# MarineRoboticsGroup/mac

Measured on AMD Instinct MI355X. Metric: frank_wolfe_iters_per_sec, higher is better.
Workload: dtype f64; 1 GPU; configs[3]: ER N=100000 ~2M candidates, chain fixed, K=10%; N=100000, m_candidates=2001737, K=200173, fixed_edges=99999, fw_iters=209, parallelism=single GPU

## Files before the change

include/machip.h:

```cpp
#ifndef MACHIP_H
#define MACHIP_H

#include <stdint.h>

#ifdef __cplusplus
extern "C" {
#endif

#define MACHIP_ABI_VERSION 16

typedef enum machip_status {
    MACHIP_OK = 0,
    MACHIP_NOT_CONVERGED = 1,
    MACHIP_DISCONNECTED = 2,
    MACHIP_BAD_ARG = 3,
    MACHIP_HIP_ERROR = 4,
    MACHIP_RCCL_ERROR = 5,
    MACHIP_NO_DEVICE = 6
} machip_status;

typedef struct machip_problem machip_problem;

typedef struct machip_solve_stats {
    int64_t lanczos_steps;
    int64_t spmv_total;
    int64_t vec_passes;
    int64_t restarts;
    int64_t nnz;
    int64_t support;
    double residual;
    double lnorm;
    double gpu_ms;
// ... 66 lines not shown
int machip_comm_mode(machip_problem* p);
int machip_shard_plan(int64_t m, int nranks, int rank, int64_t* lo, int64_t* hi, int64_t* shard);

int machip_eval_batch(machip_problem* p, int B, const double* X, double tol, int max_steps, double* lambda2,
                      int* status);

int machip_fw_sweep(machip_problem* p, int B, const int64_t* ks, const double* X0, int max_iters, double gap_tol,
                    double grad_tol, double tol, int max_steps, int warm_start, int round_decimals, double* X_out,
                    double* R_out, double* upper, double* f_traj, int* iters, int* status);

int machip_set_solver(machip_problem* p, int mode);

int machip_set_precision(machip_problem* p, int precision);

#define MACHIP_OPTION_AUTO INT64_MIN
int machip_set_option(machip_problem* p, const char* name, int64_t value);
int machip_get_option(machip_problem* p, const char* name, int64_t* value);
const char* machip_option_name(int i);

int machip_synchronize(machip_problem* p);

int machip_membench(int device, int64_t bytes, int reps, double* read_gbs, double* triad_gbs);
int machip_panel_plan(int64_t n, int64_t nnz, int maxlen, int* out12);
void machip_release_cache(void);
int machip_host_tridiag_smallest(const double* a, const double* b, int J, double* theta, double* s);
int machip_host_follow_records(const double* tri3, int J, int n, double e_target, double tiny_l, int jcap, int* points, int cap,
                               int* npoints, int* jeff, double* est);

typedef struct machip_esp machip_esp;
#define MACHIP_ESP_DENSE_INVERSE 1
#define MACHIP_ESP_MATRIX_FREE 2
#define MACHIP_ESP_SPANNING_TREE 8
#define MACHIP_ESP_EDGE_RELAX 16
#define MACHIP_ESP_EDGE_RELAX_TREE 32
int machip_esp_create(int device, int64_t n, int64_t n_fixed, const int32_t* fi, const int32_t* fj, const double* fw,
                      int64_t m, const int32_t* ci, const int32_t* cj, const double* cw, int fold, int flags, machip_esp** out);
void machip_esp_destroy(machip_esp* h);
int machip_esp_select(machip_esp* h, int nb, const int64_t* ks, int32_t* order_out, double* gain_out, double* t_ms_out);
int machip_esp_weighted_resistances(machip_esp* h, double* r_out);
int machip_esp_info(machip_esp* h, int32_t* info4, double* beta);
int machip_esp_tree_plan(int64_t n, int64_t n_fixed, const int32_t* fi, const int32_t* fj, const double* fw, int32_t* parent,
                         double* R, int32_t* pre, int32_t* end, int64_t* n_seeds, int32_t* su, int32_t* sv, double* sw);
int machip_esp_seeds(machip_esp* h, int64_t* seeds_out);

int machip_esp_relax_eval(machip_esp* h, const double* x, double* F_out, double* grad_out);
int machip_esp_relax_run(machip_esp* h, int64_t k, int max_iters, double gap_tol, double grad_tol, double* x_inout,
// ... 28 lines not shown
```

mac_amd/_lib.py:

```python
from __future__ import annotations

import ctypes as C
import os

import numpy as np

_HERE = os.path.dirname(os.path.abspath(__file__))
LIB_PATH = os.environ.get("MACHIP_LIB") or os.path.join(_HERE, "libmachip.so")

OK, NOT_CONVERGED, DISCONNECTED, BAD_ARG, HIP_ERROR, RCCL_ERROR, NO_DEVICE = range(7)
STATUS_NAMES = ["OK", "NOT_CONVERGED", "DISCONNECTED", "BAD_ARG", "HIP_ERROR", "RCCL_ERROR", "NO_DEVICE"]


class MachipError(RuntimeError):
    def __init__(self, status, msg):
        super().__init__(f"libmachip: {STATUS_NAMES[status] if 0 <= status < 7 else status}: {msg}")
        self.status = status


class NotConverged(MachipError):
    pass


class Disconnected(MachipError):
# ... 52 lines not shown
    "machip_comm_init_ipc": (C.c_int, [C.c_void_p, C.c_int, C.c_int, C.c_void_p, C.c_double]),
    "machip_comm_close_ipc": (C.c_int, [C.c_void_p]),
    "machip_comm_mode": (C.c_int, [C.c_void_p]),
    "machip_shard_plan": (C.c_int, [C.c_int64, C.c_int, C.c_int, C.POINTER(C.c_int64), C.POINTER(C.c_int64), C.POINTER(C.c_int64)]),
    "machip_eval_batch": (C.c_int, [C.c_void_p, C.c_int, _f64p, C.c_double, C.c_int, _f64p, C.POINTER(C.c_int)]),
    "machip_fw_sweep": (C.c_int, [C.c_void_p, C.c_int, C.POINTER(C.c_int64), _f64p, C.c_int, C.c_double, C.c_double, C.c_double,
                                  C.c_int, C.c_int, C.c_int, _f64p, _f64p, _f64p, _f64p, C.POINTER(C.c_int), C.POINTER(C.c_int)]),
    "machip_set_solver": (C.c_int, [C.c_void_p, C.c_int]),
    "machip_set_option": (C.c_int, [C.c_void_p, C.c_char_p, C.c_int64]),
    "machip_get_option": (C.c_int, [C.c_void_p, C.c_char_p, C.POINTER(C.c_int64)]),
    "machip_option_name": (C.c_char_p, [C.c_int]),
    "machip_comm_drop_ipc": (C.c_int, [C.c_void_p]),
    "machip_comm_drop": (C.c_int, [C.c_void_p]),
    "machip_comm_timing": (C.c_int, [C.c_void_p, _f64p, _f64p]),
    "machip_solve_mode": (C.c_int, [C.c_void_p, C.POINTER(C.c_int64)]),
    "machip_set_precision": (C.c_int, [C.c_void_p, C.c_int]),
    "machip_synchronize": (C.c_int, [C.c_void_p]),
    "machip_membench": (C.c_int, [C.c_int, C.c_int64, C.c_int, _f64p, _f64p]),
    "machip_host_tridiag_smallest": (C.c_int, [_f64p, _f64p, C.c_int, _f64p, _f64p]),
    "machip_host_follow_records": (C.c_int, [_f64p, C.c_int, C.c_int, C.c_double, C.c_double, C.c_int, C.POINTER(C.c_int), C.c_int,
                                             C.POINTER(C.c_int), C.POINTER(C.c_int), C.POINTER(C.c_double)]),
    "machip_release_cache": (None, []),
    "machip_panel_plan": (C.c_int, [C.c_int64, C.c_int64, C.c_int, C.POINTER(C.c_int)]),
    "machip_esp_create": (C.c_int, [C.c_int, C.c_int64, C.c_int64, _i32p, _i32p, _f64p, C.c_int64, _i32p, _i32p, _f64p,
                                    C.c_int, C.c_int, C.POINTER(C.c_void_p)]),
    "machip_esp_destroy": (None, [C.c_void_p]),
    "machip_esp_select": (C.c_int, [C.c_void_p, C.c_int, C.POINTER(C.c_int64), _i32p, _f64p, _f64p]),
    "machip_esp_weighted_resistances": (C.c_int, [C.c_void_p, _f64p]),
    "machip_esp_info": (C.c_int, [C.c_void_p, _i32p, C.POINTER(C.c_double)]),
    "machip_esp_tree_plan": (C.c_int, [C.c_int64, C.c_int64, _i32p, _i32p, _f64p, _i32p, _f64p, _i32p, _i32p, C.POINTER(C.c_int64),
                                       _i32p, _i32p, _f64p]),
    "machip_esp_seeds": (C.c_int, [C.c_void_p, C.POINTER(C.c_int64)]),
    "machip_esp_relax_eval": (C.c_int, [C.c_void_p, _f64p, C.POINTER(C.c_double), _f64p]),
    "machip_esp_relax_run": (C.c_int, [C.c_void_p, C.c_int64, C.c_int, C.c_double, C.c_double, _f64p, _f64p, _f64p, _f64p,
                                       C.POINTER(C.c_int), C.POINTER(C.c_double)]),
    "machip_esp_relax_inner": (C.c_int, [C.c_void_p, _f64p, _f64p, C.POINTER(C.c_double)]),
    "machip_esp_relax_info": (C.c_int, [C.c_void_p, _i32p]),
    "machip_esp_relax_gram": (C.c_int, [C.c_void_p, _f64p, C.c_int64]),
    "machip_esp_exchange": (C.c_int, [C.c_void_p, C.c_int64, _i32p, C.c_int64, C.c_double, _i32p, _i32p, _i32p, _f64p,
                                      C.POINTER(C.c_int64), C.POINTER(C.c_int32), _f64p]),
    "machip_esp_exchange_edge": (C.c_int, [C.c_void_p, C.c_int64, _i32p, C.c_int64, C.c_double, _i32p, _i32p, _i32p, _f64p,
                                           C.POINTER(C.c_int64), C.POINTER(C.c_int32), _f64p]),
    "machip_eig_create": (C.c_int, [C.c_int, C.c_int64, C.c_int64, _i32p, _i32p, _f64p, C.c_int64, _i32p, _i32p, _f64p,
                                    C.c_int, C.c_int, C.c_int, C.POINTER(C.c_void_p)]),
    "machip_eig_destroy": (None, [C.c_void_p]),
    "machip_eig_select": (C.c_int, [C.c_void_p, C.c_int64, _i32p, _f64p, _f64p]),
# ... 550 lines not shown
        os.dup2(2, 1)

    def __exit__(self, *exc):
        os.dup2(self._saved, 1)
        os.close(self._saved)


def _single_node_bootstrap():
    os.environ.setdefault("NCCL_SOCKET_IFNAME", "lo")


def comm_init_local(problems):
    lib = load()
    arr = (C.c_void_p * len(problems))(*[p._h for p in problems])
    check(lib.machip_comm_init_local(arr, len(problems)))


def shard_plan(m, nranks, rank):
    lo, hi, sh = C.c_int64(), C.c_int64(), C.c_int64()
    check(load().machip_shard_plan(int(m), int(nranks), int(rank), C.byref(lo), C.byref(hi), C.byref(sh)))
    return int(lo.value), int(hi.value), int(sh.value)


def comm_unique_id() -> bytes:
    _single_node_bootstrap()
    buf = C.create_string_buffer(128)
    lib = load()
    with _stdout_to_stderr():
        st = lib.machip_comm_unique_id(buf)
    check(st)
    return buf.raw


def fiedler_csr(indptr, indices, data, n, tol=1e-8, max_steps=0, x0=None, q=0, device=0):
    lib = load()
    indptr, indices, data = i32(indptr), i32(indices), f64(data)
    lam = C.c_double()
    v = np.empty(n)
    X = np.empty((q, n)) if q else None
    x0a = f64(x0) if x0 is not None else None
    stats = SolveStats()
    check(lib.machip_fiedler_csr(int(device), int(n), p_i32(indptr), p_i32(indices), p_f64(data), float(tol),
                                 int(max_steps), p_f64(x0a), C.byref(lam), p_f64(v), p_f64(X), int(q),
                                 C.byref(stats)))
    return lam.value, v, (X.T if X is not None else None), stats

# ... 23 lines not shown
```

mac_amd/csrc/kernels.h:

```cpp
#pragma once
#include "common.h"

namespace machip {

template <typename T>
struct CsrViewT {
    int n;
    const int* rowptr;
    const int* col;
    const T* val;
};
using CsrView = CsrViewT<double>;

struct PatternView {
    int n;
    const int* prow;
    const int* pcol;
    const int* pk;
    const double* pw;
};

struct LanState {
    int jA;
    int jB;
// ... 5 lines not shown
    int n;
    LanState* st;
    double* u;
    double* w;
    double* V;
    double* alpha;
    double* beta;
    double* l1;
    double* part_u;
    int P_u;
    double* part_a;
    int P_a;
};

constexpr int kAsmGrid = 4096;
__global__ __launch_bounds__(kBlock) void k_x_bits(const double* __restrict__ x, long m, double tol, unsigned long long* __restrict__ bits) {
    for (long i = (long)blockIdx.x * kBlock + threadIdx.x; i < m; i += (long)gridDim.x * kBlock) {
        const unsigned long long bal = __ballot(x[i] > tol);
        if ((threadIdx.x & 63) == 0) bits[i >> 6] = bal;
    }
}
__device__ __forceinline__ bool x_bit(const unsigned int* __restrict__ bits32, int k) { return (bits32[k >> 5] >> (k & 31)) & 1u; }

template <int G>
__global__ __launch_bounds__(kBlock) void k_asm_count(PatternView P, const unsigned int* __restrict__ xbits,
                                                      int rows_per_block,
                                                      int* __restrict__ cnt, int* __restrict__ blk_sum,
                                                      int* __restrict__ hsum = nullptr) {
    __shared__ int sm[4];
    constexpr int GPB = kBlock / G;
    const int lane = threadIdx.x % G, g = threadIdx.x / G;
    const int r0 = blockIdx.x * rows_per_block;
    const int r1 = min(P.n, r0 + rows_per_block);
    int local = 0, supp = 0, mx = 0;
    for (int r = r0 + g; r < r1; r += GPB) {
        const int b = P.prow[r], e = P.prow[r + 1];
        int c = 0, sc = 0;
        for (int p = b + lane; p < e; p += G) {
            const int k = P.pk[p];
            const bool cand = k >= 0;
            const bool act = cand ? x_bit(xbits, k) : true;
            c += act;
            sc += (cand && act);
        }
        c = group_sum_i<G>(c);
        sc = group_sum_i<G>(sc);
        if (lane == 0) {
            cnt[r] = c + 1;
            local += c + 1;
            supp += sc;
            mx = max(mx, c + 1);
        }
    }
    const int tot = block_sum_i(local, sm);
    const int stot = block_sum_i(supp, sm);
#pragma unroll
    for (int o = 32; o > 0; o >>= 1) mx = max(mx, __shfl_xor(mx, o, kWave));
    __syncthreads();
    if ((threadIdx.x & 63) == 0) sm[threadIdx.x >> 6] = mx;
    __syncthreads();
    if (threadIdx.x == 0) {
        blk_sum[blockIdx.x] = tot;
        blk_sum[kAsmGrid + blockIdx.x] = stot;
        const int longest = max(max(sm[0], sm[1]), max(sm[2], sm[3]));
        blk_sum[2 * kAsmGrid + blockIdx.x] = longest;
        if (hsum) {
            hsum[blockIdx.x] = tot; hsum[kAsmGrid + blockIdx.x] = stot; hsum[2 * kAsmGrid + blockIdx.x] = longest;
        }
    }
}

struct PanSpec {
    int NP = 0;
    int C = 1;
    int band = 0;
    int* ps = nullptr;
    double* bd = nullptr;
    int* bpk = nullptr;
    int* ovf = nullptr;
};

template <int G>
__global__ __launch_bounds__(kBlock) void k_asm_fill(PatternView P, const unsigned int* __restrict__ xbits, const double* __restrict__ x,
                                                     int rows_per_block,
                                                     const int* __restrict__ cnt,
                                                     const int* __restrict__ blk_sum,
                                                     int* __restrict__ rowptr, int* __restrict__ col,
                                                     double* __restrict__ val,
                                                     double* __restrict__ blk_lnorm, PanSpec S = PanSpec()) {
    extern __shared__ __attribute__((aligned(16))) char smem_raw[];
    int* s_off = reinterpret_cast<int*>(smem_raw);
    __shared__ int sm_i[4];
    __shared__ double sm_d[4];
    __shared__ int s_chunk[kBlock];
    constexpr int GPB = kBlock / G;
    const int tid = threadIdx.x;
    const int lane = tid % G, g = tid / G;
    const int r0 = blockIdx.x * rows_per_block;
    const int r1 = min(P.n, r0 + rows_per_block);
    const int nr = max(0, r1 - r0);

    int acc = 0;
    for (int b = tid; b < (int)blockIdx.x; b += kBlock) acc += blk_sum[b];
    const int base = block_sum_i(acc, sm_i);

    const int per = (nr + kBlock - 1) / kBlock;
    int csum = 0;
    for (int i = 0; i < per; ++i) {
        const int idx = tid * per + i;
        if (idx < nr) csum += cnt[r0 + idx];
    }
    {
        const int ln = tid & 63, wv = tid >> 6;
        int x = csum;
        for (int o = 1; o < 64; o <<= 1) { const int y = __shfl_up(x, o, kWave); if (ln >= o) x += y; }
        if (ln == 63) s_chunk[wv] = x;
        __syncthreads();
        int before = 0;
        for (int q = 0; q < wv; ++q) before += s_chunk[q];
        int run = before + x - csum;
        if (tid == kBlock - 1) s_off[nr] = before + x;
        for (int i = 0; i < per; ++i) {
            const int idx = tid * per + i;
            if (idx < nr) { s_off[idx] = run; run += cnt[r0 + idx]; }
        }
    }
    __syncthreads();

    double lmax = 0.0;
    for (int r = r0 + g; r < r1; r += GPB) {
        const int b = P.prow[r], e = P.prow[r + 1];
        const int out = base + s_off[r - r0];
        int pos = out + 1;
        double dsum = 0.0, asum = 0.0;
        int lastpid = 0;
        int hb = 0x7fffffff, hn = 0;
        double vl = 0.0, vu = 0.0;
        const int gbase = ((tid & 63) / G) * G;
        for (int p0 = b; p0 < e; p0 += G) {
            const int p = p0 + lane;
            const bool in = p < e;
            const int kc = in ? P.pk[p] : -1;
            const double wgt = in ? P.pw[p] : 0.0;
            const double xk = kc >= 0 ? x[kc] : 1.0;
            const bool act = in && (kc < 0 || x_bit(xbits, kc));
            const double v = act ? xk * wgt : 0.0;
            const unsigned long long bal = __ballot(act);
            unsigned long long gm;
            if (G == 64) gm = bal;
            else gm = (bal >> gbase) & ((1ull << (G & 63)) - 1ull);
            const unsigned long long below = gm & ((1ull << lane) - 1ull);
            const int before = __popcll(below);
            const int c = act ? P.pcol[p] : 0;
            if (act) { col[pos + before] = c; val[pos + before] = -v; }
            if (S.NP) {
                const int pid = act ? c / S.C : 0;
                const int src = below ? 63 - __builtin_clzll(below) : 0;
                const int got = __shfl(pid, gbase + src, kWave);
                const int ppid = below ? got : lastpid;
                if (act) {
                    const int q = pos + before;
                    for (int pp = ppid + 1; pp <= pid; ++pp) S.ps[(size_t)r * (S.NP + 1) + pp] = q;
                    if (S.band && (c == r - 1 || c == r + 1)) {
                        hb = min(hb, q); hn += 1;
                        if (c == r - 1) vl += -v; else vu += -v;
                    }
                }
                if (gm) lastpid = __shfl(pid, gbase + 63 - __builtin_clzll(gm), kWave);
            }
            pos += __popcll(gm);
            dsum += v;
            asum += fabs(v);
        }
        dsum = group_sum<G>(dsum);
        asum = group_sum<G>(asum);
        if (S.NP) {
            if (lane == 0) S.ps[(size_t)r * (S.NP + 1)] = out + 1;
            for (int pp = lastpid + 1 + lane; pp <= S.NP; pp += G) S.ps[(size_t)r * (S.NP + 1) + pp] = pos;
            if (S.band) {
                hn = group_sum_i<G>(hn);
                vl = group_sum<G>(vl); vu = group_sum<G>(vu);
#pragma unroll
                for (int o = G / 2; o > 0; o >>= 1) hb = min(hb, __shfl_xor(hb, o, kWave));
                if (lane == 0) {
                    S.bpk[r] = ((hn ? hb : pos) << 3) | min(hn, 7);
                    if (hn > 7) *S.ovf = 1;
                    S.bd[r] = dsum; S.bd[(size_t)P.n + r] = vl; S.bd[2 * (size_t)P.n + r] = vu;
                }
            }
        }
        if (lane == 0) {
            rowptr[r] = out;
            col[out] = r;
            val[out] = dsum;
            lmax = fmax(lmax, fabs(dsum) + asum);
        }
    }
    lmax = block_max(lmax, sm_d);
    if (tid == 0) {
        blk_lnorm[blockIdx.x] = lmax;
        if (blockIdx.x == gridDim.x - 1) rowptr[P.n] = base + s_off[nr];
    }
}

template <int G, class Op>
__device__ __forceinline__ void spmv_rows_vec(const CsrView& A, const double* __restrict__ x, Op& op) {
    constexpr int GPB = kBlock / G;
    const int lane = threadIdx.x % G, g = threadIdx.x / G;
    const int stride = gridDim.x * GPB;
    for (int r = blockIdx.x * GPB + g; r < A.n; r += 2 * stride) {
        const int r2 = r + stride;
        const bool two = r2 < A.n;
        const int b = A.rowptr[r], e = A.rowptr[r + 1];
        const int b2 = two ? A.rowptr[r2] : 0, e2 = two ? A.rowptr[r2 + 1] : 0;
        double acc = 0.0, acc2 = 0.0;
        int p = b + lane, q = b2 + lane;
        while (p < e || q < e2) {
            double v1 = 0.0, x1 = 0.0, v2 = 0.0, x2 = 0.0;
            if (p < e) { v1 = A.val[p]; x1 = op.gather(x, A.col[p]); }
            if (q < e2) { v2 = A.val[q]; x2 = op.gather(x, A.col[q]); }
            if (p < e) acc += v1 * x1;
            if (q < e2) acc2 += v2 * x2;
            p += G; q += G;
        }
// ... 1155 lines not shown
```

mac_amd/csrc/machip.hip:

```cpp
#include <rccl/rccl.h>
#include <unistd.h>

#include <algorithm>
#include <atomic>
#include <cmath>
#include <chrono>
#include <condition_variable>
#include <functional>
#include <future>
#include <memory>
#include <mutex>
#include <numeric>
#include <thread>
#include <vector>

#include "solver.h"
#include "esp.h"
#include "esp_free.h"
#include "esp_tree.h"
#include "esp_select.h"
#include "esp_relax.h"
#include "esp_exchange.h"
#include "esp_exchange_edge.h"
#include "eig.h"
// ... 47 lines not shown
        if (broken) return false;
        const unsigned long gen = generation;
        if (++waiting == nranks) { waiting = 0; ++generation; cv.notify_all(); return true; }
        cv.wait(lk, [&] { return generation != gen || broken; });
        return !broken;
    }
    void abort() {
        std::lock_guard<std::mutex> lk(mu);
        broken = true;
        cv.notify_all();
    }
};

struct machip_problem {
    int device = 0;
    hipStream_t stream = nullptr;
    int n = 0;
    long m = 0, m_pad = 0;
    double tol_sel = 1e-10;
    int *prow = nullptr, *pcol = nullptr, *pk = nullptr;
    double* pw = nullptr;
    long P = 0;
    int asm_G = 16, asm_rpb = 1, asm_grid = 1;
    int *ci = nullptr, *cj = nullptr;
    double* cw = nullptr;
    double *x = nullptr, *x_next = nullptr, *g = nullptr, *s = nullptr, *scratch_m = nullptr;
    int *cnt = nullptr, *blk_sum = nullptr, *rowptr = nullptr, *col = nullptr;
    double *val = nullptr, *blk_lnorm = nullptr;
    unsigned long long *xb = nullptr, *xb_next = nullptr;
    bool xb_valid = false, xb_next_valid = false;
    long nnz = 0, support = 0;
    int maxlen = 0;
    double lnorm = 0.0;
    bool assembled = false, have_vec = false, csr_only = false;
    bool band_dups_ok = true;
    unsigned int* hist = nullptr;
    SelState* sel = nullptr;
    double* part_fw = nullptr;
    int* h_int = nullptr;
    double* h_dbl = nullptr;
    int* d_hint = nullptr;
    double* d_hdbl = nullptr;
    Solver sol;
    ncclComm_t comm = nullptr;
    std::shared_ptr<LocalGroup> lgroup;
    bool first_collective_pending = false;
    hipEvent_t ev_g0 = nullptr, ev_g1 = nullptr, ev_g2 = nullptr;
    bool ev_g_valid = false;
    std::unique_ptr<IpcGroup> ipcg;
    int rank = 0, nranks = 1;
// ... 12 lines not shown
        if (hipGetDeviceProperties(&prop, device) == hipSuccess && prop.multiProcessorCount > 0) {
            const int words = (prop.multiProcessorCount + 31) / 32;
            std::vector<uint32_t> mask((size_t)words, 0xffffffffu);
            if (prop.multiProcessorCount % 32) mask.back() = (1u << (prop.multiProcessorCount % 32)) - 1u;
            if (hipExtStreamCreateWithCUMask(out, (uint32_t)words, mask.data()) == hipSuccess) return MACHIP_OK;
            (void)hipGetLastError();
        }
    }
    HIP_TRY(hipStreamCreateWithFlags(out, hipStreamNonBlocking));
    return MACHIP_OK;
}

namespace {

std::mutex g_csr_mu;
machip_problem* g_csr_cache = nullptr;

struct Slot {
    int col;
    int k;
    double w;
};

int build_pattern(machip_problem* p, int64_t nf, const int32_t* fi, const int32_t* fj, const double* fw,
                  int64_t m, const int32_t* ci, const int32_t* cj, const double* cw) {
    const Options& opt = p->sol.opt;
    const int n = p->n;
    std::vector<long> deg((size_t)n + 1, 0);
    auto chk = [&](int a, int b) { return a >= 0 && a < n && b >= 0 && b < n; };
    for (int64_t e = 0; e < nf; ++e) {
        if (!chk(fi[e], fj[e])) return fail(MACHIP_BAD_ARG, "fixed edge endpoint out of range");
        if (fi[e] != fj[e]) { deg[(size_t)fi[e]]++; deg[(size_t)fj[e]]++; }
    }
    for (int64_t e = 0; e < m; ++e) {
        if (!chk(ci[e], cj[e])) return fail(MACHIP_BAD_ARG, "candidate edge endpoint out of range");
        if (ci[e] != cj[e]) { deg[(size_t)ci[e]]++; deg[(size_t)cj[e]]++; }
    }
    std::vector<long> off((size_t)n + 1, 0);
    for (int r = 0; r < n; ++r) off[(size_t)r + 1] = off[(size_t)r] + deg[(size_t)r];
    std::vector<Slot> slots((size_t)off[(size_t)n]);
    std::vector<long> cur(off.begin(), off.end() - 1);
    for (int64_t e = 0; e < nf; ++e) {
        const int a = fi[e], b = fj[e];
        if (a == b) continue;
        slots[(size_t)cur[(size_t)a]++] = Slot{b, -1, fw[e]};
        slots[(size_t)cur[(size_t)b]++] = Slot{a, -1, fw[e]};
// ... 33 lines not shown
    }
    p->P = (long)pcol.size();
    ST_TRY(dev_alloc(&p->prow, (size_t)n + 1));
    ST_TRY(dev_alloc(&p->pcol, (size_t)p->P)); ST_TRY(dev_alloc(&p->pk, (size_t)p->P)); ST_TRY(dev_alloc(&p->pw, (size_t)p->P));
    HIP_TRY(hipMemcpyAsync(p->prow, prow.data(), sizeof(int) * ((size_t)n + 1), hipMemcpyHostToDevice, p->stream));
    if (p->P) {
        HIP_TRY(hipMemcpyAsync(p->pcol, pcol.data(), sizeof(int) * (size_t)p->P, hipMemcpyHostToDevice, p->stream));
        HIP_TRY(hipMemcpyAsync(p->pk, pk.data(), sizeof(int) * (size_t)p->P, hipMemcpyHostToDevice, p->stream));
        HIP_TRY(hipMemcpyAsync(p->pw, pw.data(), sizeof(double) * (size_t)p->P, hipMemcpyHostToDevice, p->stream));
    }
    HIP_TRY(hipStreamSynchronize(p->stream));
    const double mean = n ? (double)p->P / n : 1.0;
    int G = 4;
    while (G < 64 && G < mean * 0.75) G <<= 1;
    p->asm_G = OPT(asm_g, G);
    const int gpb = kBlock / p->asm_G;
    long nblk = std::min<long>(std::min(kAsmGrid, std::max(1, OPT(asm_maxgrid, kAsmGrid))), ((long)n + gpb - 1) / gpb);
    if (nblk < 1) nblk = 1;
    long rpb = ((long)n + nblk - 1) / nblk;
    rpb = (rpb + gpb - 1) / gpb * gpb;
    p->asm_rpb = (int)rpb;
    p->asm_grid = (int)(((long)n + rpb - 1) / rpb);
    if (p->asm_grid < 1) p->asm_grid = 1;
    if ((rpb + 1) * (long)sizeof(int) > 64 * 1024)
        return fail(MACHIP_BAD_ARG, "num_nodes above the supported 16.7 million (row-offset scan of the assembly kernel)");
    return MACHIP_OK;
}

template <int G>
void launch_asm(machip_problem* p, const PanSpec& S) {
    const PatternView P = p->pattern();
    const unsigned int* xb32 = reinterpret_cast<const unsigned int*>(p->xb);
    k_asm_count<G><<<p->asm_grid, kBlock, 0, p->stream>>>(P, xb32, p->asm_rpb, p->cnt, p->blk_sum, p->d_hint);
    const size_t lds = sizeof(int) * ((size_t)p->asm_rpb + 1);
    k_asm_fill<G><<<p->asm_grid, kBlock, lds, p->stream>>>(P, xb32, p->x, p->asm_rpb, p->cnt, p->blk_sum,
                                                           p->rowptr, p->col, p->val, p->d_hdbl, S);
}

int assemble(machip_problem* p) {
    if (p->csr_only) return fail(MACHIP_BAD_ARG, "handle wraps a caller CSR; nothing to assemble");
    PanSpec S;
    ST_TRY(p->sol.pan_spec_prepare(&S));
    if (!p->xb_valid) {
        const int grid = std::max(1, (int)std::min<long>(kMaxGrid, (p->m + kBlock - 1) / kBlock));
        k_x_bits<<<grid, kBlock, 0, p->stream>>>(p->x, p->m, p->tol_sel, p->xb);
        p->xb_valid = true;
    }
    switch (p->asm_G) {
        case 4: launch_asm<4>(p, S); break;
        case 8: launch_asm<8>(p, S); break;
        case 16: launch_asm<16>(p, S); break;
        case 32: launch_asm<32>(p, S); break;
        default: launch_asm<64>(p, S); break;
    }
    HIP_TRY(hipGetLastError());
    const int gb = p->asm_grid;
    HIP_TRY(hipStreamSynchronize(p->stream));
    long nnz = 0, supp = 0;
    int maxlen = 0;
    double ln = 0.0;
    for (int b = 0; b < gb; ++b) {
        nnz += p->h_int[b]; supp += p->h_int[kAsmGrid + b]; maxlen = std::max(maxlen, p->h_int[2 * kAsmGrid + b]);
        ln = std::max(ln, p->h_dbl[b]);
    }
    p->nnz = nnz; p->support = supp / 2; p->lnorm = ln; p->maxlen = maxlen;
    p->assembled = true;
    return MACHIP_OK;
}

int alloc_common(machip_problem* p, int vbudget_mb = 0) {
    ST_TRY(p->sol.init(p->n, p->stream, vbudget_mb));
    HIP_TRY(hipHostMalloc((void**)&p->h_int, sizeof(int) * 3 * kAsmGrid, hipHostMallocMapped));
    HIP_TRY(hipHostMalloc((void**)&p->h_dbl, sizeof(double) * std::max(4 * kMaxGrid, kAsmGrid), hipHostMallocMapped));
    HIP_TRY(hipHostGetDevicePointer((void**)&p->d_hint, p->h_int, 0));
    HIP_TRY(hipHostGetDevicePointer((void**)&p->d_hdbl, p->h_dbl, 0));
    return MACHIP_OK;
}

int select_on(machip_problem* p, const double* keys, long k, SelState* st, int prefer_high, bool hist0_done = false) {
    const Options& opt = p->sol.opt;
    const long m = p->m;
    if (k < 0) k = 0;
    if (k > m) k = m;
    if (m <= kSelSmallMax && OPT(sel_small, 1)) {
        k_sel_small<<<1, 1024, 0, p->stream>>>(keys, m, (long long)k, st, prefer_high);
        HIP_TRY(hipGetLastError());
        return MACHIP_OK;
// ... 188 lines not shown
    HIP_TRY(hipSetDevice(device));
    machip_problem* p = new machip_problem();
    p->device = device;
    p->n = (int)n;
    p->m = (long)m;
    p->m_pad = (long)m;
    p->tol_sel = min_sel_tol;
    int st = MACHIP_OK;
    auto body = [&]() -> int {
        HIP_TRY(hipStreamCreateWithFlags(&p->stream, hipStreamNonBlocking));
        ST_TRY(build_pattern(p, n_fixed, fi, fj, fw, m, ci, cj, cw));
        const size_t mp = (size_t)m + 64 * 8;
        ST_TRY(dev_alloc(&p->ci, mp)); ST_TRY(dev_alloc(&p->cj, mp)); ST_TRY(dev_alloc(&p->cw, mp));
        ST_TRY(dev_alloc(&p->x, mp)); ST_TRY(dev_alloc(&p->x_next, mp)); ST_TRY(dev_alloc(&p->g, mp)); ST_TRY(dev_alloc(&p->s, mp));
        if (m) {
            HIP_TRY(hipMemcpyAsync(p->ci, ci, sizeof(int) * (size_t)m, hipMemcpyHostToDevice, p->stream));
            HIP_TRY(hipMemcpyAsync(p->cj, cj, sizeof(int) * (size_t)m, hipMemcpyHostToDevice, p->stream));
            HIP_TRY(hipMemcpyAsync(p->cw, cw, sizeof(double) * (size_t)m, hipMemcpyHostToDevice, p->stream));
        }
        HIP_TRY(hipMemsetAsync(p->x, 0, sizeof(double) * mp, p->stream));
        HIP_TRY(hipMemsetAsync(p->g, 0, sizeof(double) * mp, p->stream));
        HIP_TRY(hipStreamSynchronize(p->stream));
        const size_t cap = (size_t)p->P + (size_t)n + 8;
        ST_TRY(dev_alloc(&p->cnt, (size_t)n + 1)); ST_TRY(dev_alloc(&p->blk_sum, 3 * kAsmGrid));
        ST_TRY(dev_alloc(&p->rowptr, (size_t)n + 1)); ST_TRY(dev_alloc(&p->col, cap)); ST_TRY(dev_alloc(&p->val, cap));
        ST_TRY(dev_alloc(&p->blk_lnorm, kAsmGrid));
        ST_TRY(dev_alloc(&p->xb, (size_t)m / 64 + 2)); ST_TRY(dev_alloc(&p->xb_next, (size_t)m / 64 + 2));
        ST_TRY(dev_alloc(&p->hist, (6 + kSelRep) * kBins)); ST_TRY(dev_alloc(&p->sel, 2)); ST_TRY(dev_alloc(&p->part_fw, 2 * kMaxGrid));
        ST_TRY(alloc_common(p));
        p->sol.csr_cap = cap;
        p->sol.pat = p->pattern();
        p->sol.pan_allowed = p->band_dups_ok;
        {
            std::vector<char> has((size_t)n, 0);
            for (int64_t e = 0; e < n_fixed; ++e) {
                const int a = std::min(fi[e], fj[e]), b = std::max(fi[e], fj[e]);
                if (a >= 0 && b < n && b == a + 1 && fw[e] > 0.0) has[(size_t)a] = 1;
            }
            long cnt = 0;
            for (int64_t i = 0; i + 1 < n; ++i) cnt += has[(size_t)i];
            p->sol.chain_like = cnt >= (long)(0.98 * (double)(n - 1));
            p->sol.chain_edges = cnt;
        }
        return MACHIP_OK;
    };
    st = body();
    if (st != MACHIP_OK) { machip_destroy(p); return st; }
    *out = p;
    return MACHIP_OK;
}

void machip_destroy(machip_problem* p) {
    if (!p) return;
    for (machip_problem* q : p->lanes) machip_destroy(q);
    p->lanes.clear();
    (void)hipSetDevice(p->device);
    if (p->stream) (void)hipStreamSynchronize(p->stream);
    if (p->is_lane) { p->prow = p->pcol = p->pk = nullptr; p->pw = nullptr; p->ci = p->cj = nullptr; p->cw = nullptr; }
    if (p->comm) (void)ncclCommDestroy(p->comm);
    if (p->lgroup) p->lgroup->abort();
    if (p->ipcg) {
        IpcGroup& G = *p->ipcg;
        if (!G.clean_exit) { k_ipc_abort<<<1, 64, 0, p->stream>>>(G.view); (void)hipStreamSynchronize(p->stream); }
        p->sol.ipc = nullptr;
        p->ipcg.reset();
    }
    p->sol.destroy();
    void* ptrs[] = {p->prow, p->pcol, p->pk, p->pw, p->ci, p->cj, p->cw, p->x, p->x_next, p->g, p->s, p->scratch_m, p->cnt,
                    p->blk_sum, p->rowptr, p->col, p->val, p->blk_lnorm, p->xb, p->xb_next, p->hist, p->sel, p->part_fw};
    for (void* q : ptrs) if (q) (void)hipFree(q);
    for (hipEvent_t e : {p->ev_g0, p->ev_g1, p->ev_g2}) if (e) (void)hipEventDestroy(e);
    if (p->h_int) (void)hipHostFree(p->h_int);
    if (p->h_dbl) (void)hipHostFree(p->h_dbl);
    if (p->stream) (void)hipStreamDestroy(p->stream);
    delete p;
}

int machip_set_x(machip_problem* p, const double* x) {
    if (!p || !x || p->csr_only) return fail(MACHIP_BAD_ARG, "machip_set_x: bad handle or NULL x");
    HIP_TRY(hipSetDevice(p->device));
    HIP_TRY(hipMemcpyAsync(p->x, x, sizeof(double) * (size_t)p->m, hipMemcpyHostToDevice, p->stream));
    HIP_TRY(hipStreamSynchronize(p->stream));
    p->assembled = false; p->xb_valid = false;
    return MACHIP_OK;
}

int machip_get_x(machip_problem* p, double* x) {
    if (!p || !x || p->csr_only) return fail(MACHIP_BAD_ARG, "machip_get_x: bad handle or NULL x");
    HIP_TRY(hipSetDevice(p->device));
    HIP_TRY(hipMemcpyAsync(x, p->x, sizeof(double) * (size_t)p->m, hipMemcpyDeviceToHost, p->stream));
    HIP_TRY(hipStreamSynchronize(p->stream));
    return MACHIP_OK;
// ... 513 lines not shown
    return 0;
}

int machip_panel_plan(int64_t n, int64_t nnz, int maxlen, int* out12) {
    if (n < 1 || n > 2000000000ll || nnz < 0 || !out12) return fail(MACHIP_BAD_ARG, "machip_panel_plan: bad argument");
    const Options& opt = default_options();
    const PanPlan pp = plan_panel(opt, (int)n, (long)nnz, maxlen, true, -1, false, OPT(stream, 1) != 0);
    out12[0] = pp.on ? 1 : 0; out12[1] = pp.NP; out12[2] = pp.C; out12[3] = pp.NB; out12[4] = pp.NTB; out12[5] = pp.TWW; out12[6] = pp.RPT; out12[7] = pp.grid2;
    out12[8] = pp.u ? 1 : 0; out12[9] = pp.LPT; out12[10] = pp.TWT; out12[11] = pp.cells;
    return MACHIP_OK;
}

#ifdef PAN_CLOCKS
extern "C" int machip_debug_pan_clocks(machip_problem* p, long long* out, int groups) {
    if (!p || !out || groups < 1 || groups > kMaxGrid || !p->sol.panv.clk) return fail(MACHIP_BAD_ARG, "machip_debug_pan_clocks: no clock buffer");
    HIP_TRY(hipSetDevice(p->device));
    HIP_TRY(hipStreamSynchronize(p->stream));
    HIP_TRY(hipMemcpy(out, p->sol.panv.clk, sizeof(long long) * 16 * (size_t)groups, hipMemcpyDeviceToHost));
    HIP_TRY(hipMemset(p->sol.panv.clk, 0, sizeof(long long) * 16 * (size_t)kMaxGrid));
    return MACHIP_OK;
}
#endif

int machip_shard_plan(int64_t m, int nranks, int rank, int64_t* lo, int64_t* hi, int64_t* shard) {
    if (m < 0 || nranks < 1 || rank < 0 || rank >= nranks || !lo || !hi || !shard) return fail(MACHIP_BAD_ARG, "machip_shard_plan: bad argument");
    long a, b, c;
    shard_plan((long)m, nranks, rank, &a, &b, &c);
    *lo = a; *hi = b; *shard = c;
    return MACHIP_OK;
}

namespace {
int make_lane(machip_problem* p, machip_problem** out) {
    machip_problem* q = new machip_problem();
    q->is_lane = true;
    q->device = p->device; q->n = p->n; q->m = p->m; q->m_pad = p->m; q->tol_sel = p->tol_sel;
    q->prow = p->prow; q->pcol = p->pcol; q->pk = p->pk; q->pw = p->pw; q->P = p->P;
    q->asm_G = p->asm_G; q->asm_rpb = p->asm_rpb; q->asm_grid = p->asm_grid;
    q->ci = p->ci; q->cj = p->cj; q->cw = p->cw;
    auto body = [&]() -> int {
        ST_TRY(create_lane_stream(p->sol.opt, q->device, &q->stream));
        ST_TRY(dev_alloc(&q->x, (size_t)q->m + 64));
        const size_t cap = (size_t)q->P + (size_t)q->n + 8;
        ST_TRY(dev_alloc(&q->cnt, (size_t)q->n + 1)); ST_TRY(dev_alloc(&q->blk_sum, 3 * kAsmGrid));
        ST_TRY(dev_alloc(&q->rowptr, (size_t)q->n + 1)); ST_TRY(dev_alloc(&q->col, cap)); ST_TRY(dev_alloc(&q->val, cap));
        ST_TRY(dev_alloc(&q->blk_lnorm, kAsmGrid));
        ST_TRY(dev_alloc(&q->xb, (size_t)q->m / 64 + 2)); ST_TRY(dev_alloc(&q->xb_next, (size_t)q->m / 64 + 2));
        const Options& opt = p->sol.opt;
        q->sol.opt = opt;
        ST_TRY(alloc_common(q, std::max(16, OPT(lane_vbudget_mb, std::max(16, OPT(vbudget_mb, 4096) / 8)))));
        q->sol.csr_cap = cap;
        q->sol.pat = q->pattern();
        q->sol.pan_allowed = p->sol.pan_allowed;
        q->sol.chain_like = p->sol.chain_like; q->sol.chain_edges = p->sol.chain_edges;
        return MACHIP_OK;
    };
    const int st = body();
    if (st != MACHIP_OK) { machip_destroy(q); return st; }
    *out = q;
    return MACHIP_OK;
}

int ensure_lane_fw(machip_problem* q) {
    if (q->lane_fw_ready) return MACHIP_OK;
    const size_t mp = (size_t)q->m + 64 * 8;
    if (!q->x_next) ST_TRY(dev_alloc(&q->x_next, mp));
    if (!q->g) ST_TRY(dev_alloc(&q->g, mp));
// ... 569 lines not shown
```

Before: 133.7 iter/s.

## Replace per-row count pass with slot bitmask and prefix marks in assembly

The count kernel now scans pattern slots linearly, producing a per-64-slot active bitmask and word prefix counts instead of per-row counts. The fill kernel derives each row's output offset and each entry's position from these marks with popcount, removing the large row-offset shared-memory scan and its node-count limit. Fill also unrolls two slot groups per iteration, prefetches the next row's bounds, and computes longest-row stats itself. This trades row-granular counting for slot-granular bitmasks, adding extra mark lookups per entry during fill.

```diff
diff --git a/include/machip.h b/include/machip.h
--- a/include/machip.h
+++ b/include/machip.h
@@ -7,7 +7,7 @@
 extern "C" {
 #endif
 
-#define MACHIP_ABI_VERSION 16
+#define MACHIP_ABI_VERSION 17
 
 typedef enum machip_status {
     MACHIP_OK = 0,
@@ -120,6 +120,7 @@
 
 int machip_membench(int device, int64_t bytes, int reps, double* read_gbs, double* triad_gbs);
 int machip_panel_plan(int64_t n, int64_t nnz, int maxlen, int* out12);
+int machip_asm_mark_plan(int64_t slots, int* out3);
 void machip_release_cache(void);
 int machip_host_tridiag_smallest(const double* a, const double* b, int J, double* theta, double* s);
 int machip_host_follow_records(const double* tri3, int J, int n, double e_target, double tiny_l, int jcap, int* points, int cap,
diff --git a/mac_amd/_lib.py b/mac_amd/_lib.py
--- a/mac_amd/_lib.py
+++ b/mac_amd/_lib.py
@@ -98,6 +98,7 @@
                                              C.POINTER(C.c_int), C.POINTER(C.c_int), C.POINTER(C.c_double)]),
     "machip_release_cache": (None, []),
     "machip_panel_plan": (C.c_int, [C.c_int64, C.c_int64, C.c_int, C.POINTER(C.c_int)]),
+    "machip_asm_mark_plan": (C.c_int, [C.c_int64, C.POINTER(C.c_int)]),
     "machip_esp_create": (C.c_int, [C.c_int, C.c_int64, C.c_int64, _i32p, _i32p, _f64p, C.c_int64, _i32p, _i32p, _f64p,
                                     C.c_int, C.c_int, C.POINTER(C.c_void_p)]),
     "machip_esp_destroy": (None, [C.c_void_p]),
@@ -694,6 +695,12 @@
     return int(lo.value), int(hi.value), int(sh.value)
 
 
+def asm_mark_plan(slots):
+    out = (C.c_int * 3)()
+    check(load().machip_asm_mark_plan(int(slots), out))
+    return int(out[0]), int(out[1]), int(out[2])
+
+
 def comm_unique_id() -> bytes:
     _single_node_bootstrap()
     buf = C.create_string_buffer(128)
diff --git a/mac_amd/csrc/kernels.h b/mac_amd/csrc/kernels.h
--- a/mac_amd/csrc/kernels.h
+++ b/mac_amd/csrc/kernels.h
@@ -51,52 +51,79 @@
 }
 __device__ __forceinline__ bool x_bit(const unsigned int* __restrict__ bits32, int k) { return (bits32[k >> 5] >> (k & 31)) & 1u; }
 
-template <int G>
-__global__ __launch_bounds__(kBlock) void k_asm_count(PatternView P, const unsigned int* __restrict__ xbits,
-                                                      int rows_per_block,
-                                                      int* __restrict__ cnt, int* __restrict__ blk_sum,
-                                                      int* __restrict__ hsum = nullptr) {
+constexpr int kMarkGrid = kAsmGrid;
+constexpr int kMarkUnroll = 8;
+__global__ __launch_bounds__(kBlock) void k_asm_count(const int* __restrict__ pk, int nslots, const unsigned int* __restrict__ xbits,
+                                                      int lg, int nwords,
+                                                      unsigned long long* __restrict__ sb, int* __restrict__ sbp,
+                                                      int* __restrict__ blk_sum, int* __restrict__ hsum = nullptr) {
     __shared__ int sm[4];
-    constexpr int GPB = kBlock / G;
-    const int lane = threadIdx.x % G, g = threadIdx.x / G;
-    const int r0 = blockIdx.x * rows_per_block;
-    const int r1 = min(P.n, r0 + rows_per_block);
-    int local = 0, supp = 0, mx = 0;
-    for (int r = r0 + g; r < r1; r += GPB) {
-        const int b = P.prow[r], e = P.prow[r + 1];
-        int c = 0, sc = 0;
-        for (int p = b + lane; p < e; p += G) {
-            const int k = P.pk[p];
-            const bool cand = k >= 0;
-            const bool act = cand ? x_bit(xbits, k) : true;
-            c += act;
-            sc += (cand && act);
-        }
-        c = group_sum_i<G>(c);
-        sc = group_sum_i<G>(sc);
-        if (lane == 0) {
-            cnt[r] = c + 1;
-            local += c + 1;
-            supp += sc;
-            mx = max(mx, c + 1);
-        }
-    }
-    const int tot = block_sum_i(local, sm);
-    const int stot = block_sum_i(supp, sm);
-#pragma unroll
-    for (int o = 32; o > 0; o >>= 1) mx = max(mx, __shfl_xor(mx, o, kWave));
-    __syncthreads();
-    if ((threadIdx.x & 63) == 0) sm[threadIdx.x >> 6] = mx;
-    __syncthreads();
+    __shared__ int sm_c[4];
+    const int ln = threadIdx.x & 63, wv = threadIdx.x >> 6;
+    const int wpb = 1 << lg;
+    const int wpw = min(64, wpb >> 2);
+    const int w0 = blockIdx.x << lg;
+    const int wend = min(nwords, w0 + wpb);
+    int carry = 0, cands = 0;
+    for (int c0 = w0; c0 < wend; c0 += 4 * wpw) {
+        const int wbeg = c0 + wv * wpw;
+        unsigned long long mine = 0ull;
+        int minec = 0;
+        for (int t0 = 0; t0 < wpw; t0 += kMarkUnroll) {
+            int k[kMarkUnroll];
+            unsigned int xw[kMarkUnroll];
+            bool in[kMarkUnroll];
+#pragma unroll
+            for (int u = 0; u < kMarkUnroll; ++u) {
+                const long p = (long)(wbeg + t0 + u) * 64 + ln;
+                in[u] = t0 + u < wpw && p < (long)nslots;
+                k[u] = pk[in[u] ? p : 0];
+            }
+#pragma unroll
+            for (int u = 0; u < kMarkUnroll; ++u) {
+                if (!in[u]) k[u] = -1;
+                xw[u] = xbits[(k[u] >= 0 ? k[u] : 0) >> 5];
+            }
+#pragma unroll
+            for (int u = 0; u < kMarkUnroll; ++u) {
+                const bool cand = k[u] >= 0;
+                const bool act = in[u] && (!cand || ((xw[u] >> (k[u] & 31)) & 1u));
+                const unsigned long long bal = __ballot(act);
+                const unsigned long long balc = __ballot(cand && act);
+                if (ln == t0 + u) { mine = bal; minec = __popcll(balc); }
+            }
+        }
+        const int w = wbeg + ln;
+        const bool own = ln < wpw && w < wend;
+        const int pc = __popcll(mine);
+        int inc = pc;
+        for (int o = 1; o < 64; o <<= 1) { const int y = __shfl_up(inc, o, kWave); if (ln >= o) inc += y; }
+        __syncthreads();
+        if (ln == 63) sm[wv] = inc;
+        __syncthreads();
+        int before = 0;
+        for (int q = 0; q < wv; ++q) before += sm[q];
+        if (own) { sb[w] = mine; sbp[w] = carry + before + inc - pc; }
+        carry += (sm[0] + sm[1]) + (sm[2] + sm[3]);
+        cands += minec;
+    }
+    const int stot = block_sum_i(cands, sm_c);
     if (threadIdx.x == 0) {
-        blk_sum[blockIdx.x] = tot;
+        blk_sum[blockIdx.x] = carry;
         blk_sum[kAsmGrid + blockIdx.x] = stot;
-        const int longest = max(max(sm[0], sm[1]), max(sm[2], sm[3]));
-        blk_sum[2 * kAsmGrid + blockIdx.x] = longest;
-        if (hsum) {
-            hsum[blockIdx.x] = tot; hsum[kAsmGrid + blockIdx.x] = stot; hsum[2 * kAsmGrid + blockIdx.x] = longest;
-        }
-    }
+        if (hsum) { hsum[blockIdx.x] = carry; hsum[kAsmGrid + blockIdx.x] = stot; }
+    }
+}
+
+struct MarkView {
+    int lg = 2;
+    int nblk = 1;
+    const unsigned long long* sb = nullptr;
+    const int* sbp = nullptr;
+    const int* blk_sum = nullptr;
+};
+__device__ __forceinline__ int mark_before(const int* s_base, int lg, int s, unsigned long long word, int wprefix) {
+    return s_base[(s >> 6) >> lg] + wprefix + __popcll(word & ((1ull << (s & 63)) - 1ull));
 }
 
 struct PanSpec {
@@ -109,97 +136,116 @@
     int* ovf = nullptr;
 };
 
+constexpr int kFillU = 2;
 template <int G>
-__global__ __launch_bounds__(kBlock) void k_asm_fill(PatternView P, const unsigned int* __restrict__ xbits, const double* __restrict__ x,
-                                                     int rows_per_block,
-                                                     const int* __restrict__ cnt,
-                                                     const int* __restrict__ blk_sum,
+__global__ __launch_bounds__(kBlock) void k_asm_fill(PatternView P, const double* __restrict__ x,
+                                                     int rows_per_block, MarkView M,
                                                      int* __restrict__ rowptr, int* __restrict__ col,
                                                      double* __restrict__ val,
-                                                     double* __restrict__ blk_lnorm, PanSpec S = PanSpec()) {
-    extern __shared__ __attribute__((aligned(16))) char smem_raw[];
-    int* s_off = reinterpret_cast<int*>(smem_raw);
+                                                     double* __restrict__ blk_lnorm, int* __restrict__ blk_longest,
+                                                     PanSpec S = PanSpec()) {
+    __shared__ __attribute__((aligned(16))) int s_base[kMarkGrid];
     __shared__ int sm_i[4];
     __shared__ double sm_d[4];
-    __shared__ int s_chunk[kBlock];
     constexpr int GPB = kBlock / G;
+    constexpr int kPer = kMarkGrid / kBlock;
     const int tid = threadIdx.x;
     const int lane = tid % G, g = tid / G;
     const int r0 = blockIdx.x * rows_per_block;
     const int r1 = min(P.n, r0 + rows_per_block);
-    const int nr = max(0, r1 - r0);
-
-    int acc = 0;
-    for (int b = tid; b < (int)blockIdx.x; b += kBlock) acc += blk_sum[b];
-    const int base = block_sum_i(acc, sm_i);
-
-    const int per = (nr + kBlock - 1) / kBlock;
-    int csum = 0;
-    for (int i = 0; i < per; ++i) {
-        const int idx = tid * per + i;
-        if (idx < nr) csum += cnt[r0 + idx];
-    }
+
+    int r = r0 + g;
+    int b = 0, e = 0;
+    if (r < r1) { b = P.prow[r]; e = P.prow[r + 1]; }
+
     {
+        int t[kPer];
+        int csum = 0;
+#pragma unroll
+        for (int i = 0; i < kPer; ++i) {
+            const int idx = tid * kPer + i;
+            const int v = M.blk_sum[idx];
+            t[i] = idx < M.nblk ? v : 0;
+            csum += t[i];
+        }
         const int ln = tid & 63, wv = tid >> 6;
-        int x = csum;
-        for (int o = 1; o < 64; o <<= 1) { const int y = __shfl_up(x, o, kWave); if (ln >= o) x += y; }
-        if (ln == 63) s_chunk[wv] = x;
-        __syncthreads();
-        int before = 0;
-        for (int q = 0; q < wv; ++q) before += s_chunk[q];
-        int run = before + x - csum;
-        if (tid == kBlock - 1) s_off[nr] = before + x;
-        for (int i = 0; i < per; ++i) {
-            const int idx = tid * per + i;
-            if (idx < nr) { s_off[idx] = run; run += cnt[r0 + idx]; }
-        }
+        int inc = csum;
+        for (int o = 1; o < 64; o <<= 1) { const int y = __shfl_up(inc, o, kWave); if (ln >= o) inc += y; }
+        if (ln == 63) sm_i[wv] = inc;
+        __syncthreads();
+        int run = inc - csum;
+        for (int q = 0; q < wv; ++q) run += sm_i[q];
+#pragma unroll
+        for (int i = 0; i < kPer; ++i) { s_base[tid * kPer + i] = run; run += t[i]; }
     }
     __syncthreads();
 
     double lmax = 0.0;
-    for (int r = r0 + g; r < r1; r += GPB) {
-        const int b = P.prow[r], e = P.prow[r + 1];
-        const int out = base + s_off[r - r0];
-        int pos = out + 1;
+    int longest = 0;
+    const int gbase = ((tid & 63) / G) * G;
+    for (; r < r1; r += GPB) {
+        const int rn = r + GPB;
+        int bn = 0, en = 0;
+        if (rn < r1) { bn = P.prow[rn]; en = P.prow[rn + 1]; }
+        const int Ab = mark_before(s_base, M.lg, b, M.sb[b >> 6], M.sbp[b >> 6]);
+        const int Ae = mark_before(s_base, M.lg, e, M.sb[e >> 6], M.sbp[e >> 6]);
+        const int out = r + Ab;
+        const int pos = out + 1 + (Ae - Ab);
         double dsum = 0.0, asum = 0.0;
         int lastpid = 0;
         int hb = 0x7fffffff, hn = 0;
         double vl = 0.0, vu = 0.0;
-        const int gbase = ((tid & 63) / G) * G;
-        for (int p0 = b; p0 < e; p0 += G) {
-            const int p = p0 + lane;
-            const bool in = p < e;
-            const int kc = in ? P.pk[p] : -1;
-            const double wgt = in ? P.pw[p] : 0.0;
-            const double xk = kc >= 0 ? x[kc] : 1.0;
-            const bool act = in && (kc < 0 || x_bit(xbits, kc));
-            const double v = act ? xk * wgt : 0.0;
-            const unsigned long long bal = __ballot(act);
-            unsigned long long gm;
-            if (G == 64) gm = bal;
-            else gm = (bal >> gbase) & ((1ull << (G & 63)) - 1ull);
-            const unsigned long long below = gm & ((1ull << lane) - 1ull);
-            const int before = __popcll(below);
-            const int c = act ? P.pcol[p] : 0;
-            if (act) { col[pos + before] = c; val[pos + before] = -v; }
-            if (S.NP) {
-                const int pid = act ? c / S.C : 0;
-                const int src = below ? 63 - __builtin_clzll(below) : 0;
-                const int got = __shfl(pid, gbase + src, kWave);
-                const int ppid = below ? got : lastpid;
-                if (act) {
-                    const int q = pos + before;
-                    for (int pp = ppid + 1; pp <= pid; ++pp) S.ps[(size_t)r * (S.NP + 1) + pp] = q;
-                    if (S.band && (c == r - 1 || c == r + 1)) {
-                        hb = min(hb, q); hn += 1;
-                        if (c == r - 1) vl += -v; else vu += -v;
+        for (int p0 = b; p0 < e; p0 += kFillU * G) {
+            int sl[kFillU], kc[kFillU], cc[kFillU], wp[kFillU];
+            double wg[kFillU], xv[kFillU];
+            unsigned long long sw[kFillU];
+#pragma unroll
+            for (int u = 0; u < kFillU; ++u) {
+                const int p = p0 + u * G + lane;
+                sl[u] = p < e ? p : b;
+                kc[u] = P.pk[sl[u]];
+                wg[u] = P.pw[sl[u]];
+                cc[u] = P.pcol[sl[u]];
+                sw[u] = M.sb[sl[u] >> 6];
+                wp[u] = M.sbp[sl[u] >> 6];
+            }
+#pragma unroll
+            for (int u = 0; u < kFillU; ++u) {
+                const int p = p0 + u * G + lane;
+                const bool act = p < e && ((sw[u] >> (p & 63)) & 1ull);
+                xv[u] = act && kc[u] >= 0 ? x[kc[u]] : 1.0;
+            }
+#pragma unroll
+            for (int u = 0; u < kFillU; ++u) {
+                const int p = p0 + u * G + lane;
+                const bool act = p < e && ((sw[u] >> (p & 63)) & 1ull);
+                const double xk = xv[u];
+                const double v = act ? xk * wg[u] : 0.0;
+                const int q = out + 1 + (mark_before(s_base, M.lg, sl[u], sw[u], wp[u]) - Ab);
+                const int c = act ? cc[u] : 0;
+                if (act) { col[q] = c; val[q] = -v; }
+                if (S.NP) {
+                    const unsigned long long bal = __ballot(act);
+                    unsigned long long gm;
+                    if (G == 64) gm = bal;
+                    else gm = (bal >> gbase) & ((1ull << (G & 63)) - 1ull);
+                    const unsigned long long below = gm & ((1ull << lane) - 1ull);
+                    const int pid = act ? c / S.C : 0;
+                    const int src = below ? 63 - __builtin_clzll(below) : 0;
+                    const int got = __shfl(pid, gbase + src, kWave);
+                    const int ppid = below ? got : lastpid;
+                    if (act) {
+                        for (int pp = ppid + 1; pp <= pid; ++pp) S.ps[(size_t)r * (S.NP + 1) + pp] = q;
+                        if (S.band && (c == r - 1 || c == r + 1)) {
+                            hb = min(hb, q); hn += 1;
+                            if (c == r - 1) vl += -v; else vu += -v;
+                        }
                     }
+                    if (gm) lastpid = __shfl(pid, gbase + 63 - __builtin_clzll(gm), kWave);
                 }
-                if (gm) lastpid = __shfl(pid, gbase + 63 - __builtin_clzll(gm), kWave);
-            }
-            pos += __popcll(gm);
-            dsum += v;
-            asum += fabs(v);
+                dsum += v;
+                asum += fabs(v);
+            }
         }
         dsum = group_sum<G>(dsum);
         asum = group_sum<G>(asum);
@@ -224,11 +270,19 @@
             val[out] = dsum;
             lmax = fmax(lmax, fabs(dsum) + asum);
         }
+        longest = max(longest, pos - out);
+        b = bn; e = en;
     }
     lmax = block_max(lmax, sm_d);
+#pragma unroll
+    for (int o = 32; o > 0; o >>= 1) longest = max(longest, __shfl_xor(longest, o, kWave));
+    __syncthreads();
+    if ((tid & 63) == 0) sm_i[tid >> 6] = longest;
+    __syncthreads();
     if (tid == 0) {
         blk_lnorm[blockIdx.x] = lmax;
-        if (blockIdx.x == gridDim.x - 1) rowptr[P.n] = base + s_off[nr];
+        blk_longest[blockIdx.x] = max(max(sm_i[0], sm_i[1]), max(sm_i[2], sm_i[3]));
+        if (r1 == P.n) rowptr[P.n] = P.n + s_base[M.nblk - 1] + M.blk_sum[M.nblk - 1];
     }
 }
 
diff --git a/mac_amd/csrc/machip.hip b/mac_amd/csrc/machip.hip
--- a/mac_amd/csrc/machip.hip
+++ b/mac_amd/csrc/machip.hip
@@ -93,10 +93,12 @@
     double* pw = nullptr;
     long P = 0;
     int asm_G = 16, asm_rpb = 1, asm_grid = 1;
+    int mark_lg = 2, mark_grid = 1, mark_words = 1;
     int *ci = nullptr, *cj = nullptr;
     double* cw = nullptr;
     double *x = nullptr, *x_next = nullptr, *g = nullptr, *s = nullptr, *scratch_m = nullptr;
-    int *cnt = nullptr, *blk_sum = nullptr, *rowptr = nullptr, *col = nullptr;
+    unsigned long long* sb = nullptr;
+    int *sbp = nullptr, *blk_sum = nullptr, *rowptr = nullptr, *col = nullptr;
     double *val = nullptr, *blk_lnorm = nullptr;
     unsigned long long *xb = nullptr, *xb_next = nullptr;
     bool xb_valid = false, xb_next_valid = false;
@@ -155,6 +157,13 @@
     double w;
 };
 
+void plan_marks(long slots, int* lg, int* grid, int* words) {
+    const long w = slots / 64 + 1;
+    int l = 2;
+    while (((w + (1l << l) - 1) >> l) > kMarkGrid) ++l;
+    *lg = l; *grid = (int)((w + (1l << l) - 1) >> l); *words = (int)w;
+}
+
 int build_pattern(machip_problem* p, int64_t nf, const int32_t* fi, const int32_t* fj, const double* fw,
                   int64_t m, const int32_t* ci, const int32_t* cj, const double* cw) {
     const Options& opt = p->sol.opt;
@@ -234,8 +243,7 @@
     p->asm_rpb = (int)rpb;
     p->asm_grid = (int)(((long)n + rpb - 1) / rpb);
     if (p->asm_grid < 1) p->asm_grid = 1;
-    if ((rpb + 1) * (long)sizeof(int) > 64 * 1024)
-        return fail(MACHIP_BAD_ARG, "num_nodes above the supported 16.7 million (row-offset scan of the assembly kernel)");
+    plan_marks(p->P, &p->mark_lg, &p->mark_grid, &p->mark_words);
     return MACHIP_OK;
 }
 
@@ -243,10 +251,11 @@
 void launch_asm(machip_problem* p, const PanSpec& S) {
     const PatternView P = p->pattern();
     const unsigned int* xb32 = reinterpret_cast<const unsigned int*>(p->xb);
-    k_asm_count<G><<<p->asm_grid, kBlock, 0, p->stream>>>(P, xb32, p->asm_rpb, p->cnt, p->blk_sum, p->d_hint);
-    const size_t lds = sizeof(int) * ((size_t)p->asm_rpb + 1);
-    k_asm_fill<G><<<p->asm_grid, kBlock, lds, p->stream>>>(P, xb32, p->x, p->asm_rpb, p->cnt, p->blk_sum,
-                                                           p->rowptr, p->col, p->val, p->d_hdbl, S);
+    k_asm_count<<<p->mark_grid, kBlock, 0, p->stream>>>(P.pk, (int)p->P, xb32, p->mark_lg, p->mark_words, p->sb, p->sbp, p->blk_sum, p->d_hint);
+    MarkView M;
+    M.lg = p->mark_lg; M.nblk = p->mark_grid; M.sb = p->sb; M.sbp = p->sbp; M.blk_sum = p->blk_sum;
+    k_asm_fill<G><<<p->asm_grid, kBlock, 0, p->stream>>>(P, p->x, p->asm_rpb, M, p->rowptr, p->col, p->val,
+                                                         p->d_hdbl, p->d_hint + 2 * kAsmGrid, S);
 }
 
 int assemble(machip_problem* p) {
@@ -271,10 +280,12 @@
     long nnz = 0, supp = 0;
     int maxlen = 0;
     double ln = 0.0;
+    for (int b = 0; b < p->mark_grid; ++b) { nnz += p->h_int[b]; supp += p->h_int[kAsmGrid + b]; }
     for (int b = 0; b < gb; ++b) {
-        nnz += p->h_int[b]; supp += p->h_int[kAsmGrid + b]; maxlen = std::max(maxlen, p->h_int[2 * kAsmGrid + b]);
+        maxlen = std::max(maxlen, p->h_int[2 * kAsmGrid + b]);
         ln = std::max(ln, p->h_dbl[b]);
     }
+    nnz += p->n;
     p->nnz = nnz; p->support = supp / 2; p->lnorm = ln; p->maxlen = maxlen;
     p->assembled = true;
     return MACHIP_OK;
@@ -509,7 +520,7 @@
         HIP_TRY(hipMemsetAsync(p->g, 0, sizeof(double) * mp, p->stream));
         HIP_TRY(hipStreamSynchronize(p->stream));
         const size_t cap = (size_t)p->P + (size_t)n + 8;
-        ST_TRY(dev_alloc(&p->cnt, (size_t)n + 1)); ST_TRY(dev_alloc(&p->blk_sum, 3 * kAsmGrid));
+        ST_TRY(dev_alloc(&p->sb, (size_t)p->mark_words)); ST_TRY(dev_alloc(&p->sbp, (size_t)p->mark_words)); ST_TRY(dev_alloc(&p->blk_sum, 3 * kAsmGrid));
         ST_TRY(dev_alloc(&p->rowptr, (size_t)n + 1)); ST_TRY(dev_alloc(&p->col, cap)); ST_TRY(dev_alloc(&p->val, cap));
         ST_TRY(dev_alloc(&p->blk_lnorm, kAsmGrid));
         ST_TRY(dev_alloc(&p->xb, (size_t)m / 64 + 2)); ST_TRY(dev_alloc(&p->xb_next, (size_t)m / 64 + 2));
@@ -553,8 +564,8 @@
         p->ipcg.reset();
     }
     p->sol.destroy();
-    void* ptrs[] = {p->prow, p->pcol, p->pk, p->pw, p->ci, p->cj, p->cw, p->x, p->x_next, p->g, p->s, p->scratch_m, p->cnt,
-                    p->blk_sum, p->rowptr, p->col, p->val, p->blk_lnorm, p->xb, p->xb_next, p->hist, p->sel, p->part_fw};
+    void* ptrs[] = {p->prow, p->pcol, p->pk, p->pw, p->ci, p->cj, p->cw, p->x, p->x_next, p->g, p->s, p->scratch_m, p->sb,
+                    p->sbp, p->blk_sum, p->rowptr, p->col, p->val, p->blk_lnorm, p->xb, p->xb_next, p->hist, p->sel, p->part_fw};
     for (void* q : ptrs) if (q) (void)hipFree(q);
     for (hipEvent_t e : {p->ev_g0, p->ev_g1, p->ev_g2}) if (e) (void)hipEventDestroy(e);
     if (p->h_int) (void)hipHostFree(p->h_int);
@@ -1114,6 +1125,14 @@
 }
 #endif
 
+int machip_asm_mark_plan(int64_t slots, int* out3) {
+    if (slots < 0 || slots > 2000000000ll || !out3) return fail(MACHIP_BAD_ARG, "machip_asm_mark_plan: bad argument");
+    int lg, grid, words;
+    plan_marks((long)slots, &lg, &grid, &words);
+    out3[0] = 1 << lg; out3[1] = grid; out3[2] = words;
+    return MACHIP_OK;
+}
+
 int machip_shard_plan(int64_t m, int nranks, int rank, int64_t* lo, int64_t* hi, int64_t* shard) {
     if (m < 0 || nranks < 1 || rank < 0 || rank >= nranks || !lo || !hi || !shard) return fail(MACHIP_BAD_ARG, "machip_shard_plan: bad argument");
     long a, b, c;
@@ -1129,12 +1148,13 @@
     q->device = p->device; q->n = p->n; q->m = p->m; q->m_pad = p->m; q->tol_sel = p->tol_sel;
     q->prow = p->prow; q->pcol = p->pcol; q->pk = p->pk; q->pw = p->pw; q->P = p->P;
     q->asm_G = p->asm_G; q->asm_rpb = p->asm_rpb; q->asm_grid = p->asm_grid;
+    q->mark_lg = p->mark_lg; q->mark_grid = p->mark_grid; q->mark_words = p->mark_words;
     q->ci = p->ci; q->cj = p->cj; q->cw = p->cw;
     auto body = [&]() -> int {
         ST_TRY(create_lane_stream(p->sol.opt, q->device, &q->stream));
         ST_TRY(dev_alloc(&q->x, (size_t)q->m + 64));
         const size_t cap = (size_t)q->P + (size_t)q->n + 8;
-        ST_TRY(dev_alloc(&q->cnt, (size_t)q->n + 1)); ST_TRY(dev_alloc(&q->blk_sum, 3 * kAsmGrid));
+        ST_TRY(dev_alloc(&q->sb, (size_t)q->mark_words)); ST_TRY(dev_alloc(&q->sbp, (size_t)q->mark_words)); ST_TRY(dev_alloc(&q->blk_sum, 3 * kAsmGrid));
         ST_TRY(dev_alloc(&q->rowptr, (size_t)q->n + 1)); ST_TRY(dev_alloc(&q->col, cap)); ST_TRY(dev_alloc(&q->val, cap));
         ST_TRY(dev_alloc(&q->blk_lnorm, kAsmGrid));
         ST_TRY(dev_alloc(&q->xb, (size_t)q->m / 64 + 2)); ST_TRY(dev_alloc(&q->xb_next, (size_t)q->m / 64 + 2));
```

Result: no change. 133.7 iter/s, median of 2 (+0.0%).
